# luk036/ellalgo-rs

Hardware: AMD Instinct MI355X
Metric: ellipsoid updates/sec at n=16384; achieved HBM GB/s vs peak (higher is better)
Workload: dtype f64

## Files before the change

### ellalgo-rs_amd/csrc/ell_kernels.hpp

```cpp
#pragma once

#include <hip/hip_runtime.h>

#include "ellcalc_device.hpp"

namespace ellhip {

struct CutParams {
    int kind;
    int has_b1;
    double b0;
    double b1;
};

struct DevState {
    double kappa;
    double tsq;
    double omega;
    double ratio;
    double rho_over_omega;
    double scale;
    int status;
    int apply;
    int halted;
// ... 743 lines not shown
__global__ __launch_bounds__(256) void k_apply_mfma(double* __restrict__ Q, long long ld, long long n, long long nrows,
                                                    long long row0, const double* __restrict__ pend,
                                                    const double* __restrict__ cpend, const DevState* __restrict__ st) {
    static_assert(NP % 8 == 0, "rank of the update: a multiple of 8 (k = 4 per MFMA, whole pairs per staging thread)");
    constexpr int KS = NP / 4;
    constexpr int SPT = NP / 8;
    __shared__ double sh_v[2][NP][APM_ROWS];
    (void)st;
    const int tid = threadIdx.x, lane = tid & 63, wave = tid >> 6;
    const long long strip = (long long)gridDim.x - 1 - blockIdx.x;
    const long long lr0 = strip * APM_ROWS;
    if (lr0 >= nrows) return;
    const long long gr0 = row0 + lr0;
    const long long glast = (lr0 + APM_ROWS <= nrows ? lr0 + APM_ROWS : nrows) - 1 + row0;
    long long cend = (glast / 2 + 1) * 2;
    if (cend > n) cend = n;
    const long long c_begin = (long long)blockIdx.y * APM_COLS;
    if (c_begin >= cend) return;
    const long long c_stop = (c_begin + APM_COLS < cend) ? c_begin + APM_COLS : cend;
    const long long arow = gr0 + 16 * wave + (lane & 15);
    double a[KS];
#pragma unroll
    for (int sidx = 0; sidx < KS; ++sidx) {
        const int k = 4 * sidx + (lane >> 4);
        a[sidx] = (arow <= glast) ? -(cpend[k] * pend[(long long)k * n + arow]) : 0.0;
    }
    const int sk = tid >> 5, sj = (tid & 31) * 2;
    auto fetch = [&](double2_t (&v)[SPT], long long cb) {
#pragma unroll
        for (int t = 0; t < SPT; ++t)
            v[t] = (cb + sj < n) ? *reinterpret_cast<const double2_t*>(pend + (long long)(sk + 8 * t) * n + cb + sj) : double2_t{0.0, 0.0};
    };
    auto park = [&](int buf, const double2_t (&v)[SPT]) {
#pragma unroll
        for (int t = 0; t < SPT; ++t) *reinterpret_cast<double2_t*>(&sh_v[buf][sk + 8 * t][sj]) = v[t];
    };
    int buf = 0;
    {
        double2_t v0[SPT];
        fetch(v0, c_begin);
        park(0, v0);
    }
    __syncthreads();
    double* rbase = Q + (lr0 + 16 * wave + (lane >> 4)) * ld + 2 * (lane & 15);
    auto loadq = [&](double2_t (&x)[2][4], long long cb) __attribute__((always_inline)) {
#pragma unroll
        for (int h = 0; h < 2; ++h) {
            const long long c = cb + 32 * h + 2 * (lane & 15);
#pragma unroll
            for (int i = 0; i < 4; ++i) {
                const long long grow = gr0 + 16 * wave + (lane >> 4) + 4 * i;
                const bool on = grow <= glast && c < c_stop;
                x[h][i] = on ? ld_stream<NT, double2_t>(rbase + (long long)(4 * i) * ld + cb + 32 * h) : double2_t{0.0, 0.0};
            }
        }
    };
    auto step = [&](double2_t (&x)[2][4], double2_t (&xn)[2][4], long long cb) __attribute__((always_inline)) {
        const bool more = cb + APM_ROWS < c_stop;
        double2_t vn[SPT];
        if (more) {
            loadq(xn, cb + APM_ROWS);
            fetch(vn, cb + APM_ROWS);
        }
#pragma unroll
        for (int h = 0; h < 2; ++h) {
            const long long c = cb + 32 * h + 2 * (lane & 15);
            double4_t ce = {x[h][0].x, x[h][1].x, x[h][2].x, x[h][3].x}, co = {x[h][0].y, x[h][1].y, x[h][2].y, x[h][3].y};
#pragma unroll
            for (int sidx = 0; sidx < KS; ++sidx) {
                const double2_t b = *reinterpret_cast<const double2_t*>(&sh_v[buf][4 * sidx + (lane >> 4)][32 * h + 2 * (lane & 15)]);
                ce = __builtin_amdgcn_mfma_f64_16x16x4f64(a[sidx], b.x, ce, 0, 0, 0);
                co = __builtin_amdgcn_mfma_f64_16x16x4f64(a[sidx], b.y, co, 0, 0, 0);
            }
            const double oe[4] = {ce.x, ce.y, ce.z, ce.w}, oo[4] = {co.x, co.y, co.z, co.w};
#pragma unroll
            for (int i = 0; i < 4; ++i) {
                const long long grow = gr0 + 16 * wave + (lane >> 4) + 4 * i;
                if (grow <= glast && c < c_stop)
                    *reinterpret_cast<double2_t*>(rbase + (long long)(4 * i) * ld + cb + 32 * h) = double2_t{oe[i], oo[i]};
            }
        }
        if (more) park(buf ^ 1, vn);
        __syncthreads();
        buf ^= 1;
    };
    double2_t xa[2][4], xb[2][4];
    loadq(xa, c_begin);
    for (long long cb = c_begin; cb < c_stop; cb += 2 * APM_ROWS) {
        step(xa, xb, cb);
        if (cb + APM_ROWS < c_stop) step(xb, xa, cb + APM_ROWS);
    }
}

constexpr int SMM_NV = 16;
constexpr int SMM_PITCH = 17;

__global__ __launch_bounds__(256) void k_pack_grads(const double* __restrict__ g, long long g_stride, int lv, long long n,
                                                    double* __restrict__ gT, unsigned* __restrict__ queue = nullptr,
                                                    int nvw = SMM_NV) {
    const long long i = (long long)blockIdx.x * blockDim.x + threadIdx.x;
    if (i == 0 && queue) *queue = 0u;
    if (i >= n * nvw) return;
    const long long c = i / nvw;
    const int v = (int)(i % nvw);
    gT[i] = v < lv ? g[(long long)v * g_stride + c] : 0.0;
}

__device__ __host__ __forceinline__ int pk_vec(int t, int slot) {
    return 16 * t + 8 * (slot >> 3) + 2 * (slot & 3) + ((slot >> 2) & 1);
}

__global__ __launch_bounds__(256) void k_pack_operands(const double* __restrict__ g, long long g_stride, int lv, long long n,
                                                       double* __restrict__ gP, unsigned* __restrict__ queue, int nvt,
                                                       const double* __restrict__ pend, double* __restrict__ pendP, int ks2) {
    const long long nbg = n * nvt / 32;
    if ((long long)blockIdx.x < nbg) {
        const long long idx = (long long)blockIdx.x * 256 + threadIdx.x;
        if (idx == 0 && queue) *queue = 0u;
        const long long beta = idx / (nvt * 128);
        const int rem = (int)(idx % (nvt * 128));
        const int t = rem >> 7, kb2 = (rem >> 6) & 1, lane = rem & 63;
        const int v = pk_vec(t, lane & 15);
        const long long row = 16 * beta + 8 * kb2 + (lane >> 4);
        double2_t o = {0.0, 0.0};
        if (v < lv) o = double2_t{g[(long long)v * g_stride + row], g[(long long)v * g_stride + row + 4]};
        reinterpret_cast<double2_t*>(gP)[idx] = o;
        return;
    }
    const long long idx = ((long long)blockIdx.x - nbg) * 256 + threadIdx.x;
    if (idx >= (n / 16) * ks2 * 64) return;
    const long long cblk = idx / (ks2 * 64);
    const int s2 = (int)((idx >> 6) % ks2), lane = (int)(idx & 63);
    const long long k0 = 8 * s2 + (lane >> 4), col = 16 * cblk + (lane & 15);
    reinterpret_cast<double2_t*>(pendP)[idx] = double2_t{pend[k0 * n + col], pend[(k0 + 4) * n + col]};
}

template <int NVT>
__device__ __forceinline__ void pk_load_gc(const double* __restrict__ gP, long long cb, int t, int lane, double (&gc)[4]) {
    const double2_t* p = reinterpret_cast<const double2_t*>(gP) + (((cb >> 4) * NVT + t) * 2) * 64 + lane;
    const double2_t a = p[0], b = p[64];
    gc[0] = a.x, gc[1] = a.y, gc[2] = b.x, gc[3] = b.y;
}
template <int NVT, int PITCH>
__device__ __forceinline__ void pk_stage_sgr(const double* __restrict__ gP, long long r0, double (*sgr)[PITCH]) {
    const double2_t* p = reinterpret_cast<const double2_t*>(gP) + (r0 >> 4) * (NVT * 128);
    for (int k = threadIdx.x; k < 4 * NVT * 128; k += 256) {
        const double2_t v = p[k];
        const int blk = k / (NVT * 128), t = (k >> 7) % NVT, kb2 = (k >> 6) & 1, ln = k & 63;
        const int row = 16 * blk + 8 * kb2 + (ln >> 4), col = 16 * t + (ln & 15);
        sgr[row][col] = v.x;
        sgr[row + 4][col] = v.y;
    }
}
__device__ __forceinline__ void pk_store_colsums(double* __restrict__ colpart2, long long colpart_stride, long long I, long long n,
                                                 long long c, int t, int lr, int lv, const double4_t& dc) {
    const int p0 = 8 * t + lr;
    double* q = colpart2 + 2 * ((long long)p0 * colpart_stride + I * n + c);
    if (2 * p0 < lv) *reinterpret_cast<double2_t*>(q) = double2_t{dc.x, dc.y};
    if (2 * (p0 + 4) < lv) *reinterpret_cast<double2_t*>(q + 8 * colpart_stride) = double2_t{dc.z, dc.w};
}

template <bool NT, int SEG, bool PK = false>
__device__ __forceinline__ void symm_tile(const double* __restrict__ Q, long long ld, long long n, long long row0, long long I,
                                          long long J, const double* __restrict__ gT, int lv, double* __restrict__ rowpart,
                                          double* __restrict__ colpart, long long rowpart_stride, long long colpart_stride,
                                          double (*sh)[SYMV_H * SMM_PITCH]) {
    const int lane = threadIdx.x & 63, wave = threadIdx.x >> 6;
    const int lr = lane >> 4, lc = lane & 15;
    const long long r0 = row0 + I * SYMV_H;
    const long long c0 = J * SEG;
    const bool full = c0 + SEG - 1 < r0;
    double gr[16];
    if constexpr (PK) {
#pragma unroll
        for (int jq = 0; jq < 4; ++jq) {
            double q4[4];
            pk_load_gc<1>(gT, r0 + 16 * jq, 0, lane, q4);
#pragma unroll
            for (int k = 0; k < 4; ++k) gr[4 * jq + k] = q4[k];
        }
    } else {
#pragma unroll
        for (int j = 0; j < 16; ++j) gr[j] = gT[(r0 + 4 * j + lr) * SMM_NV + lc];
    }
    double4_t dr[4];
#pragma unroll
    for (int jj = 0; jj < 4; ++jj) dr[jj] = double4_t{0.0, 0.0, 0.0, 0.0};
    const long long cend = (c0 + SEG < r0 + SYMV_H) ? c0 + SEG : r0 + SYMV_H;
    const int nblk = (int)((cend - c0) / 16);
    double* mysh = sh[wave];
    const double* qbase = Q + (r0 + lr) * ld + lc;
    for (int b = wave; b < nblk; b += 4) {
        const long long cb = c0 + 16 * (long long)b;
        double x[16], gc[4];
#pragma unroll
        for (int j = 0; j < 16; ++j) x[j] = ld_stream<NT, double>(qbase + (long long)(4 * j) * ld + cb);
        if constexpr (PK) {
            pk_load_gc<1>(gT, cb, 0, lane, gc);
        } else {
#pragma unroll
            for (int kb = 0; kb < 4; ++kb) gc[kb] = gT[(cb + 4 * kb + lr) * SMM_NV + lc];
        }
        const bool diag = !full && cb + 15 >= r0;
        double4_t dc = {0.0, 0.0, 0.0, 0.0};
        if (diag) {
#pragma unroll
            for (int j = 0; j < 16; ++j) {
                const long long r = r0 + 4 * j + lr, c = cb + lc;
                const double below = (c < r) ? x[j] : 0.0;
                dc = __builtin_amdgcn_mfma_f64_16x16x4f64(gr[j], below, dc, 0, 0, 0);
                x[j] = (c <= r) ? x[j] : 0.0;
            }
        } else {
#pragma unroll
            for (int j = 0; j < 16; ++j) dc = __builtin_amdgcn_mfma_f64_16x16x4f64(gr[j], x[j], dc, 0, 0, 0);
        }
#pragma unroll
        for (int j = 0; j < 16; ++j) mysh[(4 * j + lr) * SMM_PITCH + lc] = x[j];
#pragma unroll
        for (int jj = 0; jj < 4; ++jj)
#pragma unroll
            for (int kb = 0; kb < 4; ++kb) {
                const double t = mysh[(16 * jj + lc) * SMM_PITCH + 4 * kb + lr];
                dr[jj] = __builtin_amdgcn_mfma_f64_16x16x4f64(gc[kb], t, dr[jj], 0, 0, 0);
            }
        if constexpr (PK) {
            pk_store_colsums(colpart, colpart_stride, I, n, cb + lc, 0, lr, lv, dc);
        } else {
            const double o[4] = {dc.x, dc.y, dc.z, dc.w};
#pragma unroll
            for (int i = 0; i < 4; ++i) {
                const int v = lr + 4 * i;
                if (v < lv) colpart[(long long)v * colpart_stride + I * n + cb + lc] = o[i];
            }
        }
    }
    __syncthreads();
    double* red = &sh[0][0];
#pragma unroll
    for (int jj = 0; jj < 4; ++jj) {
        const double o[4] = {dr[jj].x, dr[jj].y, dr[jj].z, dr[jj].w};
#pragma unroll
        for (int i = 0; i < 4; ++i) red[((wave * 4 + jj) * 4 + i) * 64 + lane] = o[i];
    }
    __syncthreads();
#pragma unroll
    for (int i = 0; i < 4; ++i) {
        const int v = PK ? pk_vec(0, lr + 4 * i) : lr + 4 * i;
        const int jj = wave;
        const double s0 = red[((0 * 4 + jj) * 4 + i) * 64 + lane], s1 = red[((1 * 4 + jj) * 4 + i) * 64 + lane];
        const double s2 = red[((2 * 4 + jj) * 4 + i) * 64 + lane], s3 = red[((3 * 4 + jj) * 4 + i) * 64 + lane];
        if (v < lv) rowpart[(long long)v * rowpart_stride + J * n + r0 + 16 * jj + lc] = ((s0 + s1) + s2) + s3;
    }
}

template <bool NT, int SEG>
__global__ __launch_bounds__(256) void k_symm_mfma(const double* __restrict__ Q, long long ld, long long n, long long row0,
                                                   long long nrows, const double* __restrict__ gT, int lv,
                                                   double* __restrict__ rowpart,
                                                   double* __restrict__ colpart, long long rowpart_stride,
                                                   long long colpart_stride, const DevState* __restrict__ st) {
    __shared__ double sh[4][SYMV_H * SMM_PITCH];
    if (st->halted) return;
    const long long I = (long long)gridDim.x - 1 - blockIdx.x, J = (long long)blockIdx.y;
    const long long r0 = row0 + I * SYMV_H;
    if (r0 >= row0 + nrows || J * SEG > r0 + SYMV_H - 1) return;
    symm_tile<NT, SEG>(Q - row0 * ld, ld, n, row0, I, J, gT, lv, rowpart, colpart, rowpart_stride, colpart_stride, sh);
}

struct SymmTile {
    int I, J;
};
template <bool NT, int SEG, bool PK = false>
__global__ __launch_bounds__(256) void k_symm_mfma_q(const double* __restrict__ Q, long long ld, long long n, long long row0,
                                                     const double* __restrict__ gT, int lv, double* __restrict__ rowpart,
                                                     double* __restrict__ colpart, long long rowpart_stride,
                                                     long long colpart_stride, const DevState* __restrict__ st,
                                                     const SymmTile* __restrict__ tiles, int ntiles,
                                                     unsigned* __restrict__ queue) {
    __shared__ double sh[4][SYMV_H * SMM_PITCH];
    __shared__ int s_t;
    if (st->halted) return;
    Q -= row0 * ld;
    for (;;) {
        __syncthreads();
        if (threadIdx.x == 0) {
            const unsigned t = atomicAdd(queue, 1u);
            s_t = t < (unsigned)ntiles ? (int)t : -1;
        }
        __syncthreads();
        const int t = s_t;
        if (t < 0) return;
        symm_tile<NT, SEG, PK>(Q, ld, n, row0, (long long)tiles[t].I, (long long)tiles[t].J, gT, lv, rowpart, colpart, rowpart_stride,
                               colpart_stride, sh);
    }
}

constexpr int SMM_NV2 = 2 * SMM_NV;
template <bool NT, int SEG, bool PK = false>
__device__ __forceinline__ void symm_tile2(const double* __restrict__ Q, long long ld, long long n, long long row0, long long I,
                                           long long J, const double* __restrict__ gT, int lv, double* __restrict__ rowpart,
                                           double* __restrict__ colpart, long long rowpart_stride, long long colpart_stride,
                                           double (*sh)[SYMV_H * SMM_PITCH], double (*sgr)[SMM_NV2 + 1]) {
    const int lane = threadIdx.x & 63, wave = threadIdx.x >> 6;
    const int lr = lane >> 4, lc = lane & 15;
    const long long r0 = row0 + I * SYMV_H;
    const long long c0 = J * SEG;
    const bool full = c0 + SEG - 1 < r0;
    if constexpr (PK) {
        pk_stage_sgr<2>(gT, r0, sgr);
    } else {
        for (int k = threadIdx.x; k < SYMV_H * SMM_NV2; k += 256) sgr[k / SMM_NV2][k % SMM_NV2] = gT[(r0 + k / SMM_NV2) * SMM_NV2 + k % SMM_NV2];
    }
    __syncthreads();
    double4_t dr[2][4];
#pragma unroll
    for (int t = 0; t < 2; ++t)
#pragma unroll
        for (int jj = 0; jj < 4; ++jj) dr[t][jj] = double4_t{0.0, 0.0, 0.0, 0.0};
    const long long cend = (c0 + SEG < r0 + SYMV_H) ? c0 + SEG : r0 + SYMV_H;
    const int nblk = (int)((cend - c0) / 16);
    double* mysh = sh[wave];
    const double* qbase = Q + (r0 + lr) * ld + lc;
    for (int b = wave; b < nblk; b += 4) {
        const long long cb = c0 + 16 * (long long)b;
        double x[16], gc[2][4];
#pragma unroll
        for (int j = 0; j < 16; ++j) x[j] = ld_stream<NT, double>(qbase + (long long)(4 * j) * ld + cb);
#pragma unroll
        for (int t = 0; t < 2; ++t) {
            if constexpr (PK) {
                pk_load_gc<2>(gT, cb, t, lane, gc[t]);
            } else {
#pragma unroll
                for (int kb = 0; kb < 4; ++kb) gc[t][kb] = gT[(cb + 4 * kb + lr) * SMM_NV2 + 16 * t + lc];
            }
        }
        const bool diag = !full && cb + 15 >= r0;
        double4_t dc[2] = {double4_t{0.0, 0.0, 0.0, 0.0}, double4_t{0.0, 0.0, 0.0, 0.0}};
#pragma unroll
        for (int t = 0; t < 2; ++t)
#pragma unroll
            for (int j = 0; j < 16; ++j) {
                const long long r = r0 + 4 * j + lr, c = cb + lc;
                const double below = (!diag || c < r) ? x[j] : 0.0;
                dc[t] = __builtin_amdgcn_mfma_f64_16x16x4f64(sgr[4 * j + lr][16 * t + lc], below, dc[t], 0, 0, 0);
            }
        if (diag) {
#pragma unroll
            for (int j = 0; j < 16; ++j) {
                const long long r = r0 + 4 * j + lr, c = cb + lc;
                x[j] = (c <= r) ? x[j] : 0.0;
            }
        }
#pragma unroll
        for (int j = 0; j < 16; ++j) mysh[(4 * j + lr) * SMM_PITCH + lc] = x[j];
#pragma unroll
        for (int t = 0; t < 2; ++t)
#pragma unroll
            for (int jj = 0; jj < 4; ++jj)
#pragma unroll
                for (int kb = 0; kb < 4; ++kb) {
                    const double tv = mysh[(16 * jj + lc) * SMM_PITCH + 4 * kb + lr];
                    dr[t][jj] = __builtin_amdgcn_mfma_f64_16x16x4f64(gc[t][kb], tv, dr[t][jj], 0, 0, 0);
                }
#pragma unroll
        for (int t = 0; t < 2; ++t) {
            if constexpr (PK) {
                pk_store_colsums(colpart, colpart_stride, I, n, cb + lc, t, lr, lv, dc[t]);
            } else {
                const double o[4] = {dc[t].x, dc[t].y, dc[t].z, dc[t].w};
#pragma unroll
                for (int i = 0; i < 4; ++i) {
                    const int v = 16 * t + lr + 4 * i;
                    if (v < lv) colpart[(long long)v * colpart_stride + I * n + cb + lc] = o[i];
                }
            }
        }
    }
    __syncthreads();
    double* red = &sh[0][0];
#pragma unroll
    for (int t = 0; t < 2; ++t) {
#pragma unroll
        for (int jj = 0; jj < 4; ++jj) {
            const double o[4] = {dr[t][jj].x, dr[t][jj].y, dr[t][jj].z, dr[t][jj].w};
#pragma unroll
            for (int i = 0; i < 4; ++i) red[((wave * 4 + jj) * 4 + i) * 64 + lane] = o[i];
        }
        __syncthreads();
#pragma unroll
        for (int i = 0; i < 4; ++i) {
            const int v = PK ? pk_vec(t, lr + 4 * i) : 16 * t + lr + 4 * i;
            const int jj = wave;
            const double s0 = red[((0 * 4 + jj) * 4 + i) * 64 + lane], s1 = red[((1 * 4 + jj) * 4 + i) * 64 + lane];
            const double s2 = red[((2 * 4 + jj) * 4 + i) * 64 + lane], s3 = red[((3 * 4 + jj) * 4 + i) * 64 + lane];
            if (v < lv) rowpart[(long long)v * rowpart_stride + J * n + r0 + 16 * jj + lc] = ((s0 + s1) + s2) + s3;
        }
        __syncthreads();
    }
}

template <bool NT, int SEG, bool PK = false>
__global__ __launch_bounds__(256, 2) void k_symm_mfma_q2(const double* __restrict__ Q, long long ld, long long n, long long row0,
                                                         const double* __restrict__ gT, int lv, double* __restrict__ rowpart,
                                                         double* __restrict__ colpart, long long rowpart_stride,
                                                         long long colpart_stride, const DevState* __restrict__ st,
                                                         const SymmTile* __restrict__ tiles, int ntiles,
                                                         unsigned* __restrict__ queue) {
    __shared__ double sh[4][SYMV_H * SMM_PITCH];
    __shared__ double sgr[SYMV_H][SMM_NV2 + 1];
    __shared__ int s_t;
    if (st->halted) return;
    Q -= row0 * ld;
    for (;;) {
        __syncthreads();
        if (threadIdx.x == 0) {
            const unsigned t = atomicAdd(queue, 1u);
            s_t = t < (unsigned)ntiles ? (int)t : -1;
        }
        __syncthreads();
        const int t = s_t;
        if (t < 0) return;
        symm_tile2<NT, SEG, PK>(Q, ld, n, row0, (long long)tiles[t].I, (long long)tiles[t].J, gT, lv, rowpart, colpart,
                                rowpart_stride, colpart_stride, sh, sgr);
    }
}

template <int NP, bool NT, int SEG, bool WIDE, bool PK = false>
__device__ __forceinline__ void apply_symm_tile(double* __restrict__ Q, long long ld, long long n, long long I, long long J,
                                                const double* __restrict__ pend, const double* __restrict__ cpend,
                                                const double* __restrict__ gT, int lv, double* __restrict__ rowpart,
                                                double* __restrict__ colpart, long long rowpart_stride, long long colpart_stride,
                                                bool prod, double (*sh)[SYMV_H * SMM_PITCH], double (*sgr)[SMM_NV2 + 1],
                                                double* __restrict__ sa, const double* __restrict__ pendP) {
    constexpr int KS = NP / 4;
    constexpr int NVT = WIDE ? 2 : 1;
    constexpr int NVW = SMM_NV * NVT;
    const int lane = threadIdx.x & 63, wave = threadIdx.x >> 6;
    const int lr = lane >> 4, lc = lane & 15;
    const long long r0 = I * SYMV_H;
    const long long c0 = J * SEG;
    const bool full = c0 + SEG - 1 < r0;
    for (int e = threadIdx.x; e < 4 * KS * 64; e += 256) {
        const int q = e / (KS * 64), s = (e / 64) % KS, ln = e % 64;
        const int k = 4 * s + (ln >> 4);
        sa[((q * (KS / 2) + s / 2) * 64 + ln) * 2 + (s & 1)] = -(cpend[k] * pend[(long long)k * n + r0 + 16 * q + (ln & 15)]);
    }
    if (prod) {
        if constexpr (PK) {
            pk_stage_sgr<NVT>(gT, r0, sgr);
        } else {
            for (int k = threadIdx.x; k < SYMV_H * NVW; k += 256) sgr[k / NVW][k % NVW] = gT[(r0 + k / NVW) * NVW + k % NVW];
        }
    }
    __syncthreads();
    double4_t dr[NVT][4];
#pragma unroll
    for (int t = 0; t < NVT; ++t)
#pragma unroll
        for (int jj = 0; jj < 4; ++jj) dr[t][jj] = double4_t{0.0, 0.0, 0.0, 0.0};
    const long long cend = (c0 + SEG < r0 + SYMV_H) ? c0 + SEG : r0 + SYMV_H;
    const int nblk = (int)((cend - c0) / 16);
    double* mysh = sh[wave];
    double* qbase = Q + (r0 + lr) * ld + lc;
    const double* pbase = pend + (long long)lr * n + lc;
    for (int b = wave; b < nblk; b += 4) {
        const long long cb = c0 + 16 * (long long)b;
        double x[16], bv[KS], gc[NVT][4];
#pragma unroll
        for (int j = 0; j < 16; ++j) x[j] = ld_stream<NT, double>(qbase + (long long)(4 * j) * ld + cb);
        if constexpr (PK) {
            const double2_t* pp = reinterpret_cast<const double2_t*>(pendP) + (cb >> 4) * (KS / 2) * 64 + lane;
#pragma unroll
            for (int s2 = 0; s2 < KS / 2; ++s2) {
                const double2_t v = pp[s2 * 64];
                bv[2 * s2] = v.x, bv[2 * s2 + 1] = v.y;
            }
        } else {
#pragma unroll
            for (int s = 0; s < KS; ++s) bv[s] = pbase[(long long)(4 * s) * n + cb];
        }
        __builtin_amdgcn_sched_barrier(0);
        double4_t acc[4];
#pragma unroll
        for (int q = 0; q < 4; ++q) acc[q] = double4_t{x[4 * q], x[4 * q + 1], x[4 * q + 2], x[4 * q + 3]};
#pragma unroll
        for (int s2 = 0; s2 < KS / 2; ++s2)
#pragma unroll
            for (int q = 0; q < 4; ++q) {
                const double2_t a = *reinterpret_cast<const double2_t*>(&sa[((q * (KS / 2) + s2) * 64 + lane) * 2]);
                acc[q] = __builtin_amdgcn_mfma_f64_16x16x4f64(a.x, bv[2 * s2], acc[q], 0, 0, 0);
                acc[q] = __builtin_amdgcn_mfma_f64_16x16x4f64(a.y, bv[2 * s2 + 1], acc[q], 0, 0, 0);
                if (q == 3) __builtin_amdgcn_sched_barrier(0);
            }
#pragma unroll
        for (int q = 0; q < 4; ++q) {
            x[4 * q] = acc[q].x;
            x[4 * q + 1] = acc[q].y;
            x[4 * q + 2] = acc[q].z;
            x[4 * q + 3] = acc[q].w;
        }
#pragma unroll
        for (int j = 0; j < 16; ++j) qbase[(long long)(4 * j) * ld + cb] = x[j];
        if (!prod) continue;
        __builtin_amdgcn_sched_barrier(0);
#pragma unroll
        for (int t = 0; t < NVT; ++t) {
            if constexpr (PK) {
                pk_load_gc<NVT>(gT, cb, t, lane, gc[t]);
            } else {
#pragma unroll
                for (int kb = 0; kb < 4; ++kb) gc[t][kb] = gT[(cb + 4 * kb + lr) * NVW + 16 * t + lc];
            }
        }
        const bool diag = !full && cb + 15 >= r0;
        double4_t dc[NVT];
#pragma unroll
        for (int t = 0; t < NVT; ++t) {
            dc[t] = double4_t{0.0, 0.0, 0.0, 0.0};
#pragma unroll
            for (int j = 0; j < 16; ++j) {
                const long long r = r0 + 4 * j + lr, c = cb + lc;
                const double below = (!diag || c < r) ? x[j] : 0.0;
                dc[t] = __builtin_amdgcn_mfma_f64_16x16x4f64(sgr[4 * j + lr][16 * t + lc], below, dc[t], 0, 0, 0);
            }
        }
        if (diag) {
#pragma unroll
            for (int j = 0; j < 16; ++j) {
                const long long r = r0 + 4 * j + lr, c = cb + lc;
                x[j] = (c <= r) ? x[j] : 0.0;
            }
        }
#pragma unroll
        for (int j = 0; j < 16; ++j) mysh[(4 * j + lr) * SMM_PITCH + lc] = x[j];
#pragma unroll
        for (int t = 0; t < NVT; ++t)
#pragma unroll
            for (int jj = 0; jj < 4; ++jj)
#pragma unroll
                for (int kb = 0; kb < 4; ++kb) {
                    const double tv = mysh[(16 * jj + lc) * SMM_PITCH + 4 * kb + lr];
                    dr[t][jj] = __builtin_amdgcn_mfma_f64_16x16x4f64(gc[t][kb], tv, dr[t][jj], 0, 0, 0);
                }
#pragma unroll
        for (int t = 0; t < NVT; ++t) {
            if constexpr (PK) {
                pk_store_colsums(colpart, colpart_stride, I, n, cb + lc, t, lr, lv, dc[t]);
            } else {
                const double o[4] = {dc[t].x, dc[t].y, dc[t].z, dc[t].w};
#pragma unroll
                for (int i = 0; i < 4; ++i) {
                    const int v = 16 * t + lr + 4 * i;
                    if (v < lv) colpart[(long long)v * colpart_stride + I * n + cb + lc] = o[i];
                }
            }
        }
    }
    if (!prod) return;
    __syncthreads();
    double* red = &sh[0][0];
#pragma unroll
    for (int t = 0; t < NVT; ++t) {
#pragma unroll
        for (int jj = 0; jj < 4; ++jj) {
            const double o[4] = {dr[t][jj].x, dr[t][jj].y, dr[t][jj].z, dr[t][jj].w};
#pragma unroll
            for (int i = 0; i < 4; ++i) red[((wave * 4 + jj) * 4 + i) * 64 + lane] = o[i];
        }
        __syncthreads();
#pragma unroll
        for (int i = 0; i < 4; ++i) {
            const int v = PK ? pk_vec(t, lr + 4 * i) : 16 * t + lr + 4 * i;
            const int jj = wave;
            const double s0 = red[((0 * 4 + jj) * 4 + i) * 64 + lane], s1 = red[((1 * 4 + jj) * 4 + i) * 64 + lane];
            const double s2 = red[((2 * 4 + jj) * 4 + i) * 64 + lane], s3 = red[((3 * 4 + jj) * 4 + i) * 64 + lane];
            if (v < lv) rowpart[(long long)v * rowpart_stride + J * n + r0 + 16 * jj + lc] = ((s0 + s1) + s2) + s3;
        }
        __syncthreads();
    }
}

template <int NP, bool NT, int SEG, bool WIDE, bool PK = false>
__global__ __launch_bounds__(256, 2) void k_apply_symm_q(double* __restrict__ Q, long long ld, long long n,
                                                         const double* __restrict__ pend, const double* __restrict__ cpend,
                                                         const double* __restrict__ gT, int lv, double* __restrict__ rowpart,
                                                         double* __restrict__ colpart, long long rowpart_stride,
                                                         long long colpart_stride, const DevState* __restrict__ st,
                                                         const SymmTile* __restrict__ tiles, int ntiles,
                                                         unsigned* __restrict__ queue,
                                                         const double* __restrict__ pendP = nullptr) {
    static_assert(NP % 8 == 0, "k-steps taken in pairs");
    __shared__ double sh[4][SYMV_H * SMM_PITCH];
    __shared__ double sgr[SYMV_H][SMM_NV2 + 1];
    __shared__ double sa[SYMV_H * NP];
    __shared__ int s_t;
    const bool prod = !st->halted;
    for (;;) {
        __syncthreads();
        if (threadIdx.x == 0) {
            const unsigned t = atomicAdd(queue, 1u);
            s_t = t < (unsigned)ntiles ? (int)t : -1;
        }
        __syncthreads();
        const int t = s_t;
        if (t < 0) return;
        apply_symm_tile<NP, NT, SEG, WIDE, PK>(Q, ld, n, (long long)tiles[t].I, (long long)tiles[t].J, pend, cpend, gT, lv, rowpart,
                                               colpart, rowpart_stride, colpart_stride, prod, sh, sgr, sa, pendP);
    }
}

constexpr int PUB_WGS = 16;
__global__ __launch_bounds__(256) void k_publish(const DevState* __restrict__ st, const double* __restrict__ xc, long long n,
                                                 LiveMirror* __restrict__ m, double* __restrict__ h_xc,
                                                 unsigned long long seq, unsigned* __restrict__ arrived) {
    __shared__ int last;
    const long long n2 = n / 2;
    for (long long i = (long long)blockIdx.x * 256 + threadIdx.x; i < n2; i += (long long)gridDim.x * 256)
        *reinterpret_cast<double2_t*>(h_xc + 2 * i) = *reinterpret_cast<const double2_t*>(xc + 2 * i);
    if ((n & 1) && blockIdx.x == 0 && threadIdx.x == 0) h_xc[n - 1] = xc[n - 1];
    __threadfence_system();
    __syncthreads();
    if (threadIdx.x == 0) {
        const unsigned old = __hip_atomic_fetch_add(arrived, 1u, __ATOMIC_ACQ_REL, __HIP_MEMORY_SCOPE_AGENT);
        last = (old + 1 == gridDim.x);
        if (last) __hip_atomic_store(arrived, 0u, __ATOMIC_RELAXED, __HIP_MEMORY_SCOPE_AGENT);
    }
    __syncthreads();
    if (!last) return;
    if (threadIdx.x < (int)(sizeof(DevState) / sizeof(long long)))
        reinterpret_cast<long long*>(&m->st)[threadIdx.x] = reinterpret_cast<const long long*>(st)[threadIdx.x];
    __threadfence_system();
    __syncthreads();
    if (threadIdx.x == 0) __hip_atomic_store(&m->seq, seq, __ATOMIC_RELEASE, __HIP_MEMORY_SCOPE_SYSTEM);
}

constexpr int STAGE_WGS = 32;
__global__ __launch_bounds__(256) void k_stage(const double* __restrict__ h_src, double* __restrict__ dst, long long n) {
    const long long n2 = n / 2;
    for (long long i = (long long)blockIdx.x * 256 + threadIdx.x; i < n2; i += (long long)gridDim.x * 256)
        *reinterpret_cast<double2_t*>(dst + 2 * i) = *reinterpret_cast<const double2_t*>(h_src + 2 * i);
    if ((n & 1) && blockIdx.x == 0 && threadIdx.x == 0) dst[n - 1] = h_src[n - 1];
}

__global__ __launch_bounds__(256) void k_pend_reset(double* __restrict__ pend, double* __restrict__ cpend,
                                                    long long total, DevState* __restrict__ st) {
    for (long long i = (long long)blockIdx.x * blockDim.x + threadIdx.x; i < total;
         i += (long long)gridDim.x * blockDim.x)
        pend[i] = 0.0;
    if (blockIdx.x == 0 && threadIdx.x < MAXPEND) cpend[threadIdx.x] = 0.0;
    if (blockIdx.x == 0 && threadIdx.x == 0) st->npend = 0;
}

#ifndef ELLHIP_SCALAR_SLICE
#define ELLHIP_SCALAR_SLICE 1024
#endif
__host__ __device__ inline int scalar_groups(long long n) {
    long long g = n / ELLHIP_SCALAR_SLICE;
    if (g < 1) g = 1;
    if (g > 64) g = 64;
    return (int)g;
}
__host__ __device__ inline long long scalar_slice(long long n) {
    const long long g = scalar_groups(n);
    long long m = (n + g - 1) / g;
    return (m + 1) & ~1LL;
}

__global__ __launch_bounds__(256) void k_scalar_dot(long long n, const double* __restrict__ g,
                                                    const double* __restrict__ gt,
                                                    double* __restrict__ partial, DevState* __restrict__ st) {
    __shared__ double red[4];
    const int tid = threadIdx.x;
    const int halted = st->halted;
    if (blockIdx.x == 0 && tid == 0) {
        st->halted_in = halted;
        st->kappa_in = st->kappa;
    }
    if (halted) return;
    const long long m = scalar_slice(n);
    const long long lo = (long long)blockIdx.x * m;
    const long long hi = (lo + m < n) ? lo + m : n;
    double s = 0.0;
    for (long long i = lo + tid; i < hi; i += 256) s += g[i] * gt[i];
    s = wave_allreduce_sum(s);
    if ((tid & 63) == 0) red[tid >> 6] = s;
    __syncthreads();
    if (tid == 0) partial[blockIdx.x] = ((red[0] + red[1]) + red[2]) + red[3];
}

__global__ __launch_bounds__(256) void k_scalar_apply(long long n, const double* __restrict__ gt,
                                                      double* __restrict__ xc,
                                                      const double* __restrict__ partial,
                                                      DevState* __restrict__ st, EllCalcDev calc,
                                                      const CutParams* __restrict__ cp_dev, CutParams cp_val,
                                                      int no_defer_trick, int queue_mode,
                                                      int* __restrict__ q_status, double* __restrict__ q_tsq) {
    __shared__ double bc_roo;
    __shared__ int bc_status;
    const int tid = threadIdx.x;
    const bool lead = blockIdx.x == 0;
    if (st->halted_in) {
        if (lead && tid == 0 && q_status) {
            *q_status = ST_UNKNOWN;
            *q_tsq = st->tsq;
        }
        return;
    }
    if (tid == 0) {
        const int G = scalar_groups(n);
        double omega = 0.0;
        for (int b = 0; b < G; ++b) omega += partial[b];
        const double kappa = st->kappa_in;
        const double tsq = kappa * omega;
        Coef cf;
        const CutParams cp = cp_dev ? *cp_dev : cp_val;
        const int status = calc.dispatch(cp.kind, cp.b0, cp.has_b1, cp.b1, tsq, cf);
        double roo = 0.0;
        if (status == ST_SUCCESS) roo = cf.rho / omega;
        if (lead) {
            st->tsq = tsq;
            st->omega = omega;
            st->status = status;
            if (status == ST_SUCCESS) {
                st->rho_over_omega = roo;
                st->ratio = cf.sigma / omega;
                const double knew = kappa * cf.delta;
                if (no_defer_trick) {
                    st->scale = knew;
                    st->kappa = 1.0;
                } else {
                    st->scale = 1.0;
                    st->kappa = knew;
                }
                st->apply = 1;
            } else {
                st->apply = 0;
            }
            queue_bookkeeping(st, status, tsq, queue_mode);
            if (q_status) {
                *q_status = status;
                *q_tsq = tsq;
            }
        }
        bc_roo = roo;
        bc_status = status;
    }
    __syncthreads();
    if (bc_status != ST_SUCCESS) return;
    const double roo = bc_roo;
    const long long m = scalar_slice(n);
    const long long lo = (long long)blockIdx.x * m;
    const long long hi = (lo + m < n) ? lo + m : n;
    for (long long i = lo + tid; i < hi; i += 256) xc[i] = xc[i] - roo * gt[i];
}

constexpr int SC_LP_ROWS = 128;

template <int NP>
__global__ __launch_bounds__(256) void k_scalar_dot_def(long long n, const double* __restrict__ g,
// ... 393 lines not shown
```

Measured before the change: 35300.

## Software-pipeline Q block loads and repack sgr for vector LDS reads in symm kernels

```diff
diff --git a/ellalgo-rs_amd/csrc/ell_kernels.hpp b/ellalgo-rs_amd/csrc/ell_kernels.hpp
--- a/ellalgo-rs_amd/csrc/ell_kernels.hpp
+++ b/ellalgo-rs_amd/csrc/ell_kernels.hpp
@@ -919,10 +919,50 @@
         sgr[row + 4][col] = v.y;
     }
 }
+constexpr int PL_ROTATE = 1, PL_SGR2 = 2, PL_ACC = 4;
+constexpr int SYMM2_PL = PL_ROTATE | PL_SGR2;
+constexpr int APPLY_SYMM_PL = PL_ROTATE | PL_SGR2 | PL_ACC;
+__device__ __forceinline__ void pl_drain_vmem() {
+    __builtin_amdgcn_s_waitcnt(0x0F70);
+}
+template <bool B>
+struct PlConst {
+    static constexpr bool value = B;
+};
+struct PlValue {
+    bool value;
+};
+__device__ __forceinline__ int pl_wave() { return __builtin_amdgcn_readfirstlane((int)(threadIdx.x >> 6)); }
+
+template <int NVT>
+__device__ __forceinline__ void pk_stage_sgr2(const double* __restrict__ gP, long long r0, double* __restrict__ sgr2) {
+    const double2_t* p = reinterpret_cast<const double2_t*>(gP) + (r0 >> 4) * (NVT * 128);
+    for (int k = threadIdx.x; k < 4 * NVT * 128; k += 256) {
+        const int blk = k / (NVT * 128), t = (k >> 7) % NVT, kb2 = (k >> 6) & 1, ln = k & 63;
+        reinterpret_cast<double2_t*>(sgr2)[(t * 8 + 2 * blk + kb2) * 64 + ln] = p[k];
+    }
+}
+template <int NVT>
+__device__ __forceinline__ void stage_sgr2(const double* __restrict__ gT, long long r0, double* __restrict__ sgr2) {
+    constexpr int NVW = SMM_NV * NVT;
+    for (int k = threadIdx.x; k < SYMV_H * NVW; k += 256) {
+        const int row = k / NVW, col = k % NVW;
+        sgr2[(((col >> 4) * 8 + (row >> 3)) * 64 + 16 * (row & 3) + (col & 15)) * 2 + ((row >> 2) & 1)] = gT[(r0 + row) * NVW + col];
+    }
+}
+
 __device__ __forceinline__ void pk_store_colsums(double* __restrict__ colpart2, long long colpart_stride, long long I, long long n,
                                                  long long c, int t, int lr, int lv, const double4_t& dc) {
     const int p0 = 8 * t + lr;
     double* q = colpart2 + 2 * ((long long)p0 * colpart_stride + I * n + c);
+    if (2 * p0 < lv) *reinterpret_cast<double2_t*>(q) = double2_t{dc.x, dc.y};
+    if (2 * (p0 + 4) < lv) *reinterpret_cast<double2_t*>(q + 8 * colpart_stride) = double2_t{dc.z, dc.w};
+}
+
+__device__ __forceinline__ void pk_store_colsums_at(double* __restrict__ lbase, long long colpart_stride, long long cb, int t, int lr,
+                                                    int lv, const double4_t& dc) {
+    const int p0 = 8 * t + lr;
+    double* q = lbase + 2 * ((long long)(8 * t) * colpart_stride + cb);
     if (2 * p0 < lv) *reinterpret_cast<double2_t*>(q) = double2_t{dc.x, dc.y};
     if (2 * (p0 + 4) < lv) *reinterpret_cast<double2_t*>(q + 8 * colpart_stride) = double2_t{dc.z, dc.w};
 }
@@ -1064,17 +1104,27 @@
 }
 
 constexpr int SMM_NV2 = 2 * SMM_NV;
-template <bool NT, int SEG, bool PK = false>
+template <bool NT, int SEG, bool PK = false, int PL = SYMM2_PL>
 __device__ __forceinline__ void symm_tile2(const double* __restrict__ Q, long long ld, long long n, long long row0, long long I,
                                            long long J, const double* __restrict__ gT, int lv, double* __restrict__ rowpart,
                                            double* __restrict__ colpart, long long rowpart_stride, long long colpart_stride,
                                            double (*sh)[SYMV_H * SMM_PITCH], double (*sgr)[SMM_NV2 + 1]) {
-    const int lane = threadIdx.x & 63, wave = threadIdx.x >> 6;
+    constexpr bool ROT = (PL & PL_ROTATE) != 0, SGR2 = (PL & PL_SGR2) != 0;
+    const int lane = threadIdx.x & 63, wave = ROT ? pl_wave() : (int)(threadIdx.x >> 6);
+    if constexpr ((PL & PL_ROTATE) != 0) {
+        I = __builtin_amdgcn_readfirstlane((int)I);
+        J = __builtin_amdgcn_readfirstlane((int)J);
+    }
     const int lr = lane >> 4, lc = lane & 15;
     const long long r0 = row0 + I * SYMV_H;
     const long long c0 = J * SEG;
     const bool full = c0 + SEG - 1 < r0;
-    if constexpr (PK) {
+    double* sgr2 = &sgr[0][0];
+    if constexpr (SGR2 && PK) {
+        pk_stage_sgr2<2>(gT, r0, sgr2);
+    } else if constexpr (SGR2) {
+        stage_sgr2<2>(gT, r0, sgr2);
+    } else if constexpr (PK) {
         pk_stage_sgr<2>(gT, r0, sgr);
     } else {
         for (int k = threadIdx.x; k < SYMV_H * SMM_NV2; k += 256) sgr[k / SMM_NV2][k % SMM_NV2] = gT[(r0 + k / SMM_NV2) * SMM_NV2 + k % SMM_NV2];
@@ -1089,11 +1139,19 @@
     const int nblk = (int)((cend - c0) / 16);
     double* mysh = sh[wave];
     const double* qbase = Q + (r0 + lr) * ld + lc;
+    double* cbase = colpart + 2 * ((long long)lr * colpart_stride + I * n + lc);
+    double x[16];
+    auto load_block = [&](long long cb) {
+#pragma unroll
+        for (int j = 0; j < 16; ++j) x[j] = ld_stream<NT, double>(qbase + (long long)(4 * j) * ld + cb);
+    };
+    if constexpr (ROT) {
+        if (wave < nblk) load_block(c0 + 16 * (long long)wave);
+    }
     for (int b = wave; b < nblk; b += 4) {
         const long long cb = c0 + 16 * (long long)b;
-        double x[16], gc[2][4];
-#pragma unroll
-        for (int j = 0; j < 16; ++j) x[j] = ld_stream<NT, double>(qbase + (long long)(4 * j) * ld + cb);
+        double gc[2][4];
+        if constexpr (!ROT) load_block(cb);
 #pragma unroll
         for (int t = 0; t < 2; ++t) {
             if constexpr (PK) {
@@ -1104,46 +1162,63 @@
             }
         }
         const bool diag = !full && cb + 15 >= r0;
+        const int dg = (int)(cb - r0) + lc - lr;
         double4_t dc[2] = {double4_t{0.0, 0.0, 0.0, 0.0}, double4_t{0.0, 0.0, 0.0, 0.0}};
 #pragma unroll
         for (int t = 0; t < 2; ++t)
 #pragma unroll
-            for (int j = 0; j < 16; ++j) {
-                const long long r = r0 + 4 * j + lr, c = cb + lc;
-                const double below = (!diag || c < r) ? x[j] : 0.0;
-                dc[t] = __builtin_amdgcn_mfma_f64_16x16x4f64(sgr[4 * j + lr][16 * t + lc], below, dc[t], 0, 0, 0);
+            for (int j = 0; j < 16; j += 2) {
+                const double below0 = (!diag || dg < 4 * j) ? x[j] : 0.0;
+                const double below1 = (!diag || dg < 4 * j + 4) ? x[j + 1] : 0.0;
+                double2_t a;
+                if constexpr (SGR2) a = *reinterpret_cast<const double2_t*>(&sgr2[((t * 8 + j / 2) * 64 + lane) * 2]);
+                else a = double2_t{sgr[4 * j + lr][16 * t + lc], sgr[4 * j + 4 + lr][16 * t + lc]};
+                dc[t] = __builtin_amdgcn_mfma_f64_16x16x4f64(a.x, below0, dc[t], 0, 0, 0);
+                dc[t] = __builtin_amdgcn_mfma_f64_16x16x4f64(a.y, below1, dc[t], 0, 0, 0);
             }
         if (diag) {
 #pragma unroll
-            for (int j = 0; j < 16; ++j) {
-                const long long r = r0 + 4 * j + lr, c = cb + lc;
-                x[j] = (c <= r) ? x[j] : 0.0;
-            }
+            for (int j = 0; j < 16; ++j) x[j] = (dg <= 4 * j) ? x[j] : 0.0;
         }
 #pragma unroll
         for (int j = 0; j < 16; ++j) mysh[(4 * j + lr) * SMM_PITCH + lc] = x[j];
-#pragma unroll
-        for (int t = 0; t < 2; ++t)
-#pragma unroll
-            for (int jj = 0; jj < 4; ++jj)
-#pragma unroll
-                for (int kb = 0; kb < 4; ++kb) {
-                    const double tv = mysh[(16 * jj + lc) * SMM_PITCH + 4 * kb + lr];
-                    dr[t][jj] = __builtin_amdgcn_mfma_f64_16x16x4f64(gc[t][kb], tv, dr[t][jj], 0, 0, 0);
+        auto store_colsums = [&] {
+#pragma unroll
+            for (int t = 0; t < 2; ++t) {
+                if constexpr (PK) {
+                    if constexpr (ROT) pk_store_colsums_at(cbase, colpart_stride, cb, t, lr, lv, dc[t]);
+                    else pk_store_colsums(colpart, colpart_stride, I, n, cb + lc, t, lr, lv, dc[t]);
+                } else {
+                    const double o[4] = {dc[t].x, dc[t].y, dc[t].z, dc[t].w};
+#pragma unroll
+                    for (int i = 0; i < 4; ++i) {
+                        const int v = 16 * t + lr + 4 * i;
+                        if (v < lv) colpart[(long long)v * colpart_stride + I * n + cb + lc] = o[i];
+                    }
                 }
-#pragma unroll
-        for (int t = 0; t < 2; ++t) {
-            if constexpr (PK) {
-                pk_store_colsums(colpart, colpart_stride, I, n, cb + lc, t, lr, lv, dc[t]);
-            } else {
-                const double o[4] = {dc[t].x, dc[t].y, dc[t].z, dc[t].w};
-#pragma unroll
-                for (int i = 0; i < 4; ++i) {
-                    const int v = 16 * t + lr + 4 * i;
-                    if (v < lv) colpart[(long long)v * colpart_stride + I * n + cb + lc] = o[i];
-                }
-            }
-        }
+            }
+        };
+        auto row_products = [&] {
+#pragma unroll
+            for (int t = 0; t < 2; ++t)
+#pragma unroll
+                for (int jj = 0; jj < 4; ++jj)
+#pragma unroll
+                    for (int kb = 0; kb < 4; ++kb) {
+                        const double tv = mysh[(16 * jj + lc) * SMM_PITCH + 4 * kb + lr];
+                        dr[t][jj] = __builtin_amdgcn_mfma_f64_16x16x4f64(gc[t][kb], tv, dr[t][jj], 0, 0, 0);
+                    }
+        };
+        if constexpr (ROT) {
+            __builtin_amdgcn_sched_barrier(0);
+            pl_drain_vmem();
+            store_colsums();
+            if (b + 4 < nblk) load_block(cb + 64);
+            __builtin_amdgcn_sched_barrier(0);
+        }
+        row_products();
+        if constexpr (ROT) __builtin_amdgcn_sched_barrier(0);
+        else store_colsums();
     }
     __syncthreads();
     double* red = &sh[0][0];
@@ -1168,7 +1243,7 @@
     }
 }
 
-template <bool NT, int SEG, bool PK = false>
+template <bool NT, int SEG, bool PK = false, int PL = SYMM2_PL>
 __global__ __launch_bounds__(256, 2) void k_symm_mfma_q2(const double* __restrict__ Q, long long ld, long long n, long long row0,
                                                          const double* __restrict__ gT, int lv, double* __restrict__ rowpart,
                                                          double* __restrict__ colpart, long long rowpart_stride,
@@ -1176,7 +1251,7 @@
                                                          const SymmTile* __restrict__ tiles, int ntiles,
                                                          unsigned* __restrict__ queue) {
     __shared__ double sh[4][SYMV_H * SMM_PITCH];
-    __shared__ double sgr[SYMV_H][SMM_NV2 + 1];
+    __shared__ alignas(16) double sgr[SYMV_H][SMM_NV2 + 1];
     __shared__ int s_t;
     if (st->halted) return;
     Q -= row0 * ld;
@@ -1189,12 +1264,12 @@
         __syncthreads();
         const int t = s_t;
         if (t < 0) return;
-        symm_tile2<NT, SEG, PK>(Q, ld, n, row0, (long long)tiles[t].I, (long long)tiles[t].J, gT, lv, rowpart, colpart,
+        symm_tile2<NT, SEG, PK, PL>(Q, ld, n, row0, (long long)tiles[t].I, (long long)tiles[t].J, gT, lv, rowpart, colpart,
                                 rowpart_stride, colpart_stride, sh, sgr);
     }
 }
 
-template <int NP, bool NT, int SEG, bool WIDE, bool PK = false>
+template <int NP, bool NT, int SEG, bool WIDE, bool PK = false, int PL = APPLY_SYMM_PL>
 __device__ __forceinline__ void apply_symm_tile(double* __restrict__ Q, long long ld, long long n, long long I, long long J,
                                                 const double* __restrict__ pend, const double* __restrict__ cpend,
                                                 const double* __restrict__ gT, int lv, double* __restrict__ rowpart,
@@ -1204,7 +1279,11 @@
     constexpr int KS = NP / 4;
     constexpr int NVT = WIDE ? 2 : 1;
     constexpr int NVW = SMM_NV * NVT;
-    const int lane = threadIdx.x & 63, wave = threadIdx.x >> 6;
+    const int lane = threadIdx.x & 63, wave = (PL & PL_ROTATE) ? pl_wave() : (int)(threadIdx.x >> 6);
+    if constexpr ((PL & PL_ROTATE) != 0) {
+        I = __builtin_amdgcn_readfirstlane((int)I);
+        J = __builtin_amdgcn_readfirstlane((int)J);
+    }
     const int lr = lane >> 4, lc = lane & 15;
     const long long r0 = I * SYMV_H;
     const long long c0 = J * SEG;
@@ -1214,8 +1293,14 @@
         const int k = 4 * s + (ln >> 4);
         sa[((q * (KS / 2) + s / 2) * 64 + ln) * 2 + (s & 1)] = -(cpend[k] * pend[(long long)k * n + r0 + 16 * q + (ln & 15)]);
     }
+    constexpr bool ROT = (PL & PL_ROTATE) != 0, SGR2 = (PL & PL_SGR2) != 0, ACC = (PL & PL_ACC) != 0;
+    double* sgr2 = &sgr[0][0];
     if (prod) {
-        if constexpr (PK) {
+        if constexpr (SGR2 && PK) {
+            pk_stage_sgr2<NVT>(gT, r0, sgr2);
+        } else if constexpr (SGR2) {
+            stage_sgr2<NVT>(gT, r0, sgr2);
+        } else if constexpr (PK) {
             pk_stage_sgr<NVT>(gT, r0, sgr);
         } else {
             for (int k = threadIdx.x; k < SYMV_H * NVW; k += 256) sgr[k / NVW][k % NVW] = gT[(r0 + k / NVW) * NVW + k % NVW];
@@ -1232,9 +1317,9 @@
     double* mysh = sh[wave];
     double* qbase = Q + (r0 + lr) * ld + lc;
     const double* pbase = pend + (long long)lr * n + lc;
-    for (int b = wave; b < nblk; b += 4) {
-        const long long cb = c0 + 16 * (long long)b;
-        double x[16], bv[KS], gc[NVT][4];
+    double* cbase = colpart + 2 * ((long long)lr * colpart_stride + I * n + lc);
+    double x[16], bv[KS];
+    auto load_block = [&](long long cb) {
 #pragma unroll
         for (int j = 0; j < 16; ++j) x[j] = ld_stream<NT, double>(qbase + (long long)(4 * j) * ld + cb);
         if constexpr (PK) {
@@ -1248,19 +1333,41 @@
 #pragma unroll
             for (int s = 0; s < KS; ++s) bv[s] = pbase[(long long)(4 * s) * n + cb];
         }
+    };
+    auto block_loop = [&](auto pc) __attribute__((always_inline)) {
+    if constexpr (ROT) {
+        if (wave < nblk) load_block(c0 + 16 * (long long)wave);
+    }
+    for (int b = wave; b < nblk; b += 4) {
+        const long long cb = c0 + 16 * (long long)b;
+        double gc[NVT][4];
+        if constexpr (!ROT) load_block(cb);
         __builtin_amdgcn_sched_barrier(0);
         double4_t acc[4];
 #pragma unroll
         for (int q = 0; q < 4; ++q) acc[q] = double4_t{x[4 * q], x[4 * q + 1], x[4 * q + 2], x[4 * q + 3]};
-#pragma unroll
-        for (int s2 = 0; s2 < KS / 2; ++s2)
+        if constexpr (ACC) {
 #pragma unroll
             for (int q = 0; q < 4; ++q) {
-                const double2_t a = *reinterpret_cast<const double2_t*>(&sa[((q * (KS / 2) + s2) * 64 + lane) * 2]);
-                acc[q] = __builtin_amdgcn_mfma_f64_16x16x4f64(a.x, bv[2 * s2], acc[q], 0, 0, 0);
-                acc[q] = __builtin_amdgcn_mfma_f64_16x16x4f64(a.y, bv[2 * s2 + 1], acc[q], 0, 0, 0);
-                if (q == 3) __builtin_amdgcn_sched_barrier(0);
-            }
+#pragma unroll
+                for (int s2 = 0; s2 < KS / 2; ++s2) {
+                    const double2_t a = *reinterpret_cast<const double2_t*>(&sa[((q * (KS / 2) + s2) * 64 + lane) * 2]);
+                    acc[q] = __builtin_amdgcn_mfma_f64_16x16x4f64(a.x, bv[2 * s2], acc[q], 0, 0, 0);
+                    acc[q] = __builtin_amdgcn_mfma_f64_16x16x4f64(a.y, bv[2 * s2 + 1], acc[q], 0, 0, 0);
+                }
+                __builtin_amdgcn_sched_barrier(0);
+            }
+        } else {
+#pragma unroll
+            for (int s2 = 0; s2 < KS / 2; ++s2)
+#pragma unroll
+                for (int q = 0; q < 4; ++q) {
+                    const double2_t a = *reinterpret_cast<const double2_t*>(&sa[((q * (KS / 2) + s2) * 64 + lane) * 2]);
+                    acc[q] = __builtin_amdgcn_mfma_f64_16x16x4f64(a.x, bv[2 * s2], acc[q], 0, 0, 0);
+                    acc[q] = __builtin_amdgcn_mfma_f64_16x16x4f64(a.y, bv[2 * s2 + 1], acc[q], 0, 0, 0);
+                    if (q == 3) __builtin_amdgcn_sched_barrier(0);
+                }
+        }
 #pragma unroll
         for (int q = 0; q < 4; ++q) {
             x[4 * q] = acc[q].x;
@@ -1270,7 +1377,13 @@
         }
 #pragma unroll
         for (int j = 0; j < 16; ++j) qbase[(long long)(4 * j) * ld + cb] = x[j];
-        if (!prod) continue;
+        if (!pc.value) {
+            if constexpr (ROT) {
+                __builtin_amdgcn_sched_barrier(0);
+                if (b + 4 < nblk) load_block(cb + 64);
+            }
+            continue;
+        }
         __builtin_amdgcn_sched_barrier(0);
 #pragma unroll
         for (int t = 0; t < NVT; ++t) {
@@ -1282,48 +1395,72 @@
             }
         }
         const bool diag = !full && cb + 15 >= r0;
+        const int dg = (int)(cb - r0) + lc - lr;
         double4_t dc[NVT];
 #pragma unroll
         for (int t = 0; t < NVT; ++t) {
             dc[t] = double4_t{0.0, 0.0, 0.0, 0.0};
 #pragma unroll
-            for (int j = 0; j < 16; ++j) {
-                const long long r = r0 + 4 * j + lr, c = cb + lc;
-                const double below = (!diag || c < r) ? x[j] : 0.0;
-                dc[t] = __builtin_amdgcn_mfma_f64_16x16x4f64(sgr[4 * j + lr][16 * t + lc], below, dc[t], 0, 0, 0);
+            for (int j = 0; j < 16; j += 2) {
+                const double below0 = (!diag || dg < 4 * j) ? x[j] : 0.0;
+                const double below1 = (!diag || dg < 4 * j + 4) ? x[j + 1] : 0.0;
+                double2_t a;
+                if constexpr (SGR2) a = *reinterpret_cast<const double2_t*>(&sgr2[((t * 8 + j / 2) * 64 + lane) * 2]);
+                else a = double2_t{sgr[4 * j + lr][16 * t + lc], sgr[4 * j + 4 + lr][16 * t + lc]};
+                dc[t] = __builtin_amdgcn_mfma_f64_16x16x4f64(a.x, below0, dc[t], 0, 0, 0);
+                dc[t] = __builtin_amdgcn_mfma_f64_16x16x4f64(a.y, below1, dc[t], 0, 0, 0);
             }
         }
         if (diag) {
 #pragma unroll
-            for (int j = 0; j < 16; ++j) {
-                const long long r = r0 + 4 * j + lr, c = cb + lc;
-                x[j] = (c <= r) ? x[j] : 0.0;
-            }
+            for (int j = 0; j < 16; ++j) x[j] = (dg <= 4 * j) ? x[j] : 0.0;
         }
 #pragma unroll
         for (int j = 0; j < 16; ++j) mysh[(4 * j + lr) * SMM_PITCH + lc] = x[j];
-#pragma unroll
-        for (int t = 0; t < NVT; ++t)
-#pragma unroll
-            for (int jj = 0; jj < 4; ++jj)
-#pragma unroll
-                for (int kb = 0; kb < 4; ++kb) {
-                    const double tv = mysh[(16 * jj + lc) * SMM_PITCH + 4 * kb + lr];
-                    dr[t][jj] = __builtin_amdgcn_mfma_f64_16x16x4f64(gc[t][kb], tv, dr[t][jj], 0, 0, 0);
+        auto store_colsums = [&] {
+#pragma unroll
+            for (int t = 0; t < NVT; ++t) {
+                if constexpr (PK) {
+                    if constexpr (ROT) pk_store_colsums_at(cbase, colpart_stride, cb, t, lr, lv, dc[t]);
+                    else pk_store_colsums(colpart, colpart_stride, I, n, cb + lc, t, lr, lv, dc[t]);
+                } else {
+                    const double o[4] = {dc[t].x, dc[t].y, dc[t].z, dc[t].w};
+#pragma unroll
+                    for (int i = 0; i < 4; ++i) {
+                        const int v = 16 * t + lr + 4 * i;
+                        if (v < lv) colpart[(long long)v * colpart_stride + I * n + cb + lc] = o[i];
+                    }
                 }
-#pragma unroll
-        for (int t = 0; t < NVT; ++t) {
-            if constexpr (PK) {
-                pk_store_colsums(colpart, colpart_stride, I, n, cb + lc, t, lr, lv, dc[t]);
-            } else {
-                const double o[4] = {dc[t].x, dc[t].y, dc[t].z, dc[t].w};
-#pragma unroll
-                for (int i = 0; i < 4; ++i) {
-                    const int v = 16 * t + lr + 4 * i;
-                    if (v < lv) colpart[(long long)v * colpart_stride + I * n + cb + lc] = o[i];
-                }
-            }
-        }
+            }
+        };
+        auto row_products = [&] {
+#pragma unroll
+            for (int t = 0; t < NVT; ++t)
+#pragma unroll
+                for (int jj = 0; jj < 4; ++jj)
+#pragma unroll
+                    for (int kb = 0; kb < 4; ++kb) {
+                        const double tv = mysh[(16 * jj + lc) * SMM_PITCH + 4 * kb + lr];
+                        dr[t][jj] = __builtin_amdgcn_mfma_f64_16x16x4f64(gc[t][kb], tv, dr[t][jj], 0, 0, 0);
+                    }
+        };
+        if constexpr (ROT) {
+            __builtin_amdgcn_sched_barrier(0);
+            pl_drain_vmem();
+            store_colsums();
+            if (b + 4 < nblk) load_block(cb + 64);
+            __builtin_amdgcn_sched_barrier(0);
+        }
+        row_products();
+        if constexpr (ROT) __builtin_amdgcn_sched_barrier(0);
+        else store_colsums();
+    }
+    };
+    if constexpr (ROT) {
+        if (prod) block_loop(PlConst<true>{});
+        else block_loop(PlConst<false>{});
+    } else {
+        block_loop(PlValue{prod});
     }
     if (!prod) return;
     __syncthreads();
@@ -1349,7 +1486,7 @@
     }
 }
 
-template <int NP, bool NT, int SEG, bool WIDE, bool PK = false>
+template <int NP, bool NT, int SEG, bool WIDE, bool PK = false, int PL = APPLY_SYMM_PL>
 __global__ __launch_bounds__(256, 2) void k_apply_symm_q(double* __restrict__ Q, long long ld, long long n,
                                                          const double* __restrict__ pend, const double* __restrict__ cpend,
                                                          const double* __restrict__ gT, int lv, double* __restrict__ rowpart,
@@ -1360,8 +1497,8 @@
                                                          const double* __restrict__ pendP = nullptr) {
     static_assert(NP % 8 == 0, "k-steps taken in pairs");
     __shared__ double sh[4][SYMV_H * SMM_PITCH];
-    __shared__ double sgr[SYMV_H][SMM_NV2 + 1];
-    __shared__ double sa[SYMV_H * NP];
+    __shared__ alignas(16) double sgr[SYMV_H][SMM_NV2 + 1];
+    __shared__ alignas(16) double sa[SYMV_H * NP];
     __shared__ int s_t;
     const bool prod = !st->halted;
     for (;;) {
@@ -1373,7 +1510,7 @@
         __syncthreads();
         const int t = s_t;
         if (t < 0) return;
-        apply_symm_tile<NP, NT, SEG, WIDE, PK>(Q, ld, n, (long long)tiles[t].I, (long long)tiles[t].J, pend, cpend, gT, lv, rowpart,
+        apply_symm_tile<NP, NT, SEG, WIDE, PK, PL>(Q, ld, n, (long long)tiles[t].I, (long long)tiles[t].J, pend, cpend, gT, lv, rowpart,
                                                colpart, rowpart_stride, colpart_stride, prod, sh, sgr, sa, pendP);
     }
 }
```

After: 36750, median of 6. 4.1% higher.
